# vasil-pashov/sparse_matrix_math

Hardware: AMD Instinct MI355X
Metric: CSR SpMV GB/s (% HBM peak) + BiCGStab iters/sec, 10M rows, 1/2/4/8 GPU (higher is better)
Workload: dtype f32

## Files before the change

### include/smm_hip.h

```cpp
#ifndef SMM_HIP_H
#define SMM_HIP_H

#include <stddef.h>

#ifdef __cplusplus
extern "C" {
#endif

#define SMM_HIP_VERSION_MAJOR 0
#define SMM_HIP_VERSION_MINOR 1

#define SMM_HIP_OK 0
#define SMM_HIP_ERR_INVALID (-1)
#define SMM_HIP_ERR_HIP (-2)
#define SMM_HIP_ERR_NO_DEVICE (-3)
#define SMM_HIP_ERR_PRECOND (-4)
#define SMM_HIP_ERR_NOMEM (-5)
#define SMM_HIP_ERR_COMM (-6)

#define SMM_SOLVER_SUCCESS 0
#define SMM_SOLVER_DIVERGED 1
#define SMM_SOLVER_MAX_ITERATIONS_REACHED 2

#define SMM_OP_ASSIGN 0
// ... 3 lines not shown
#define SMM_PRECOND_NONE 0
#define SMM_PRECOND_JACOBI 1
#define SMM_PRECOND_ILU0 2
#define SMM_PRECOND_SGS 3
#define SMM_PRECOND_IC0 4
#define SMM_PRECOND_BLOCK_ILU0 5
#define SMM_PRECOND_BLOCK_SGS 6

#define SMM_DTYPE_F32 0
#define SMM_DTYPE_F64 1
#define SMM_DTYPE_I64 2

#define SMM_SPMV_AUTO 0
#define SMM_SPMV_VECTOR 1
#define SMM_SPMV_STREAM 2
#define SMM_SPMV_PATTERN 3
#define SMM_PATTERN_NONE 0
#define SMM_PATTERN_MASKS 1
#define SMM_PATTERN_CODES 2
#define SMM_PATTERN_CONST 3

typedef struct smm_hip_csr smm_hip_csr;
typedef struct smm_hip_precond smm_hip_precond;
typedef void* smm_hip_stream;

int smm_hip_init(int device);
int smm_hip_shutdown(void);
const char* smm_hip_last_error(void);
int smm_hip_uses_std_fma(void);
int smm_hip_device_info(char* name, size_t name_cap, int* cus, size_t* hbm_bytes);
int smm_hip_stream_synchronize(smm_hip_stream stream);

int smm_hip_debug_fail_next_alloc(size_t min_bytes);
int smm_hip_profile_enable(int on);
int smm_hip_profile_read(double* spmv_ms, long long* spmv_launches, int reset);
int smm_hip_profile_read_waits(double* exposed_ms, long long* pairs, int reset);

int smm_hip_csr_create_f32(int rows, int cols, const int* start, const int* positions, const float* values, smm_hip_csr** out);
int smm_hip_csr_create_f64(int rows, int cols, const int* start, const int* positions, const double* values, smm_hip_csr** out);
int smm_hip_csr_create_dev_f32(int rows, int cols, const int* d_start, const int* d_positions, const float* d_values, smm_hip_csr** out);
int smm_hip_csr_create_dev_f64(int rows, int cols, const int* d_start, const int* d_positions, const double* d_values, smm_hip_csr** out);
int smm_hip_csr_destroy(smm_hip_csr* m);
int smm_hip_csr_info(const smm_hip_csr* m, int* rows, int* cols, int* nnz, int* dtype, int* first_active_start);
int smm_hip_csr_set_kernel(smm_hip_csr* m, int family, int lanes_per_row);
int smm_hip_csr_get_kernel(const smm_hip_csr* m, int* family, int* lanes_per_row);
int smm_hip_csr_tile_info(const smm_hip_csr* m, int* tiles, int* tile_nnz_cap, int* tile_max_rows, int* tile_kernel);
int smm_hip_csr_pattern_info(const smm_hip_csr* m, int* encoding, int* offsets);
int smm_hip_csr_kernel_desc(const smm_hip_csr* m, char* name, int name_cap, long long* bytes_per_launch);
int smm_hip_set_march_min_rows(long long const_diagonals_rows, long long values_read_rows);
int smm_hip_set_cg_lazy_x_min_bytes(long long bytes);
int smm_hip_set_cg_fuse_p(int on);
int smm_hip_csr_pattern_allow_const(smm_hip_csr* m, int allow);
int smm_hip_csr_pattern_slots(smm_hip_csr* m, int mode);
int smm_hip_csr_autotune(smm_hip_csr* m);

#define SMM_UPDATE_SET 0
#define SMM_UPDATE_ADD 1
int smm_hip_csr_scale_f32(smm_hip_csr* m, float alpha, smm_hip_stream stream);
int smm_hip_csr_scale_f64(smm_hip_csr* m, double alpha, smm_hip_stream stream);
int smm_hip_csr_axpy_f32(smm_hip_csr* m, float alpha, const smm_hip_csr* other, smm_hip_stream stream);
int smm_hip_csr_axpy_f64(smm_hip_csr* m, double alpha, const smm_hip_csr* other, smm_hip_stream stream);
int smm_hip_csr_zero_f32(smm_hip_csr* m, smm_hip_stream stream);
int smm_hip_csr_zero_f64(smm_hip_csr* m, smm_hip_stream stream);
int smm_hip_csr_update_entries_f32(smm_hip_csr* m, int n, const int* rows, const int* cols, const float* values, int mode, unsigned char* found);
int smm_hip_csr_update_entries_f64(smm_hip_csr* m, int n, const int* rows, const int* cols, const double* values, int mode, unsigned char* found);
int smm_hip_csr_update_entries_dev_f32(smm_hip_csr* m, int n, const int* d_rows, const int* d_cols, const float* d_values, int mode, unsigned char* d_found,
                                       smm_hip_stream stream);
int smm_hip_csr_update_entries_dev_f64(smm_hip_csr* m, int n, const int* d_rows, const int* d_cols, const double* d_values, int mode, unsigned char* d_found,
                                       smm_hip_stream stream);
int smm_hip_csr_set_values_f32(smm_hip_csr* m, const float* values);
int smm_hip_csr_set_values_f64(smm_hip_csr* m, const double* values);
int smm_hip_csr_set_values_dev_f32(smm_hip_csr* m, const float* d_values, smm_hip_stream stream);
int smm_hip_csr_set_values_dev_f64(smm_hip_csr* m, const double* d_values, smm_hip_stream stream);
int smm_hip_csr_get_values_f32(const smm_hip_csr* m, float* values);
int smm_hip_csr_get_values_f64(const smm_hip_csr* m, double* values);
int smm_hip_csr_values_changed_f32(smm_hip_csr* m, smm_hip_stream stream);
int smm_hip_csr_values_changed_f64(smm_hip_csr* m, smm_hip_stream stream);
int smm_hip_csr_same_pattern(const smm_hip_csr* a, const smm_hip_csr* b, int* same);

int smm_hip_spmv_f32(const smm_hip_csr* m, int op, const float* lhs, const float* x, float* out);
int smm_hip_spmv_f64(const smm_hip_csr* m, int op, const double* lhs, const double* x, double* out);
int smm_hip_spmv_dev_f32(const smm_hip_csr* m, int op, const float* d_lhs, const float* d_x, float* d_out, smm_hip_stream stream);
int smm_hip_spmv_dev_f64(const smm_hip_csr* m, int op, const double* d_lhs, const double* d_x, double* d_out, smm_hip_stream stream);

int smm_hip_dot_f32(int n, const float* a, const float* b, float* result);
int smm_hip_dot_f64(int n, const double* a, const double* b, double* result);
int smm_hip_dot_dev_f32(int n, const float* d_a, const float* d_b, float* d_result, smm_hip_stream stream);
int smm_hip_dot_dev_f64(int n, const double* d_a, const double* d_b, double* d_result, smm_hip_stream stream);

int smm_hip_axpy_dev_f32(int n, float a, const float* d_x, const float* d_y, float* d_out, smm_hip_stream stream);
int smm_hip_axpy_dev_f64(int n, double a, const double* d_x, const double* d_y, double* d_out, smm_hip_stream stream);

int smm_hip_cg_f32(const smm_hip_csr* a, const float* b, const float* x0, float* x, int maxIterations, float eps,
                   const smm_hip_precond* M, int* solver_status, int* iterations, float* resnorm2);
int smm_hip_cg_f64(const smm_hip_csr* a, const double* b, const double* x0, double* x, int maxIterations, double eps,
                   const smm_hip_precond* M, int* solver_status, int* iterations, double* resnorm2);
int smm_hip_cg_dev_f32(const smm_hip_csr* a, const float* d_b, const float* d_x0, float* d_x, int maxIterations, float eps,
                       const smm_hip_precond* M, smm_hip_stream stream, int* solver_status, int* iterations, float* resnorm2);
int smm_hip_cg_dev_f64(const smm_hip_csr* a, const double* d_b, const double* d_x0, double* d_x, int maxIterations, double eps,
                       const smm_hip_precond* M, smm_hip_stream stream, int* solver_status, int* iterations, double* resnorm2);

#define SMM_CG_RESIDENT_OFF 0
#define SMM_CG_RESIDENT_AUTO 1
#define SMM_CG_RESIDENT_REQUIRE 2
int smm_hip_cg_resident(int mode);

// ... 157 lines not shown
```

### sparse_matrix_math_amd/_lib.py

```python
import ctypes
import os
from ctypes import POINTER, c_char_p, c_double, c_float, c_int, c_longlong, c_size_t, c_ulonglong, c_void_p

_HERE = os.path.dirname(os.path.abspath(__file__))

SMM_HIP_OK = 0
SMM_HIP_ERR_INVALID = -1
SMM_HIP_ERR_HIP = -2
SMM_HIP_ERR_NO_DEVICE = -3
SMM_HIP_ERR_PRECOND = -4
SMM_HIP_ERR_NOMEM = -5
SMM_HIP_ERR_COMM = -6


class SmmHipError(RuntimeError):
    def __init__(self, code, message):
        super().__init__(f"libsmm_hip error {code}: {message}")
        self.code = code


def library_path(fma=False):
    if os.environ.get("SMM_HIP_LIBRARY"):
        return os.environ["SMM_HIP_LIBRARY"]
    name = "libsmm_hip_fma.so" if fma else "libsmm_hip.so"
# ... 26 lines not shown
    "smm_hip_precond_apply_spmv_dev": (c_int, [_P, _P, _P, _P]),
    "smm_hip_precond_values": (c_int, [_P, _P, c_size_t]),
    "smm_hip_gen_poisson2d_dev": (c_int, [c_int, c_int, _P, _P, _P, _P]),
    "smm_hip_gen_stencil3d_dev": (c_int, [c_int, c_int, c_int, "T", "T", "T", _P, _P, _P, _P]),
    "smm_hip_gen_banded_dev": (c_int, [c_int, c_int, c_ulonglong, c_int, "T", _P, _P, _P, _P]),
    "smm_hip_gen_banded_rows_dev": (c_int, [c_int, c_int, c_ulonglong, c_int, "T", c_int, c_int, _P, _P, _P, _P]),
    "smm_hip_spmv_fused_dev": (c_int, [_P, c_int, _P, _P, _P, c_int, _P, _P, _P]),
    "smm_hip_spmv_fused_finish_dev": (c_int, [_P, c_int, _P, _P, _P, c_int, _P, _P, _P]),
    "smm_hip_bicgstab_ws_create": (c_int, [c_int, POINTER(_P)]),
    "smm_hip_bicgstab_ws_stage": (c_int, [_P, c_int, _P, "T", _P]),
    "smm_hip_cg_ws_stage": (c_int, [_P, c_int, _P, _P, "T", _P]),
    "smm_hip_bicgstab_ws_result": (c_int, [_P, _P, POINTER(c_int), POINTER(c_int), "PT"]),
    "smm_hip_dist_csr_create_dev": (c_int, [_P, c_int, POINTER(c_int), _P, _P, _P, POINTER(_P)]),
    "smm_hip_dist_spmv_dev": (c_int, [_P, c_int, _P, _P, _P, _P]),
    "smm_hip_dist_bicgstab_dev": (c_int, [_P, _P, _P, c_int, "T", _P, _P, POINTER(c_int), POINTER(c_int), "PT"]),
    "smm_hip_dist_cg_dev": (c_int, [_P, _P, _P, _P, c_int, "T", _P, POINTER(c_int), POINTER(c_int), "PT"]),
    "smm_hip_csr_scale": (c_int, [_P, "T", _P]),
    "smm_hip_csr_axpy": (c_int, [_P, "T", _P, _P]),
    "smm_hip_csr_zero": (c_int, [_P, _P]),
    "smm_hip_csr_update_entries": (c_int, [_P, c_int, _P, _P, _P, c_int, _P]),
    "smm_hip_csr_update_entries_dev": (c_int, [_P, c_int, _P, _P, _P, c_int, _P, _P]),
    "smm_hip_csr_set_values": (c_int, [_P, _P]),
    "smm_hip_csr_set_values_dev": (c_int, [_P, _P, _P]),
    "smm_hip_csr_get_values": (c_int, [_P, _P]),
    "smm_hip_csr_values_changed": (c_int, [_P, _P]),
}



_PLAIN = {
    "smm_hip_init": (c_int, [c_int]),
    "smm_hip_shutdown": (c_int, []),
    "smm_hip_last_error": (c_char_p, []),
    "smm_hip_uses_std_fma": (c_int, []),
    "smm_hip_device_info": (c_int, [c_char_p, c_size_t, POINTER(c_int), POINTER(c_size_t)]),
    "smm_hip_stream_synchronize": (c_int, [_P]),
    "smm_hip_debug_fail_next_alloc": (c_int, [c_size_t]),
    "smm_hip_profile_enable": (c_int, [c_int]),
    "smm_hip_profile_read": (c_int, [POINTER(c_double), POINTER(c_longlong), c_int]),
    "smm_hip_profile_read_waits": (c_int, [POINTER(c_double), POINTER(c_longlong), c_int]),
    "smm_hip_csr_destroy": (c_int, [_P]),
    "smm_hip_csr_info": (c_int, [_P, POINTER(c_int), POINTER(c_int), POINTER(c_int), POINTER(c_int), POINTER(c_int)]),
    "smm_hip_csr_set_kernel": (c_int, [_P, c_int, c_int]),
    "smm_hip_csr_get_kernel": (c_int, [_P, POINTER(c_int), POINTER(c_int)]),
    "smm_hip_csr_autotune": (c_int, [_P]),
    "smm_hip_csr_tile_info": (c_int, [_P, POINTER(c_int), POINTER(c_int), POINTER(c_int), POINTER(c_int)]),
    "smm_hip_csr_pattern_info": (c_int, [_P, POINTER(c_int), POINTER(c_int)]),
    "smm_hip_csr_kernel_desc": (c_int, [_P, c_char_p, c_int, POINTER(c_longlong)]),
    "smm_hip_set_march_min_rows": (c_int, [c_longlong, c_longlong]),
    "smm_hip_set_cg_lazy_x_min_bytes": (c_int, [c_longlong]),
    "smm_hip_set_cg_fuse_p": (c_int, [c_int]),
    "smm_hip_csr_pattern_allow_const": (c_int, [_P, c_int]),
    "smm_hip_csr_pattern_slots": (c_int, [_P, c_int]),
    "smm_hip_csr_same_pattern": (c_int, [_P, _P, POINTER(c_int)]),
    "smm_hip_precond_create": (c_int, [_P, c_int, POINTER(_P)]),
    "smm_hip_precond_create_block": (c_int, [_P, c_int, c_int, POINTER(_P)]),
    "smm_hip_precond_create_block_capped": (c_int, [_P, c_int, c_int, c_int, POINTER(_P)]),
    "smm_hip_precond_block_level_cap": (c_int, [_P, POINTER(c_int)]),
    "smm_hip_precond_create_block_ex": (c_int, [_P, c_int, c_int, c_int, c_int, POINTER(_P)]),
    "smm_hip_precond_block_rows": (c_int, [_P, _P, c_size_t, _P]),
    "smm_hip_precond_block_record_bytes": (c_int, [_P, POINTER(c_int), POINTER(c_int), POINTER(c_int)]),
    "smm_hip_precond_block_count": (c_int, [_P, POINTER(c_int)]),
    "smm_hip_precond_block_bounds": (c_int, [_P, _P, c_size_t]),
    "smm_hip_precond_destroy": (c_int, [_P]),
    "smm_hip_precond_set_sweep": (c_int, [_P, c_int]),
    "smm_hip_precond_take_error": (c_int, [_P, _P]),
    "smm_hip_precond_info": (c_int, [_P, POINTER(c_int), POINTER(c_int), POINTER(c_int)]),
    "smm_hip_gen_poisson2d_nnz": (c_longlong, [c_int, c_int]),
    "smm_hip_gen_stencil3d_nnz": (c_longlong, [c_int, c_int, c_int]),
    "smm_hip_gen_banded_nnz": (c_longlong, [c_int, c_int, c_ulonglong, c_int]),
    "smm_hip_gen_banded_row_start": (c_longlong, [c_int, c_int, c_ulonglong, c_int, c_int]),
    "smm_hip_partials_count": (c_int, []),
    "smm_hip_finish_len": (c_int, []),
    "smm_hip_finish_totals_offset": (c_int, []),
    "smm_hip_cg_resident": (c_int, [c_int]),
    "smm_hip_bicgstab_resident": (c_int, [c_int]),
    "smm_hip_bicgstab_ws_destroy": (c_int, [_P]),
    "smm_hip_cg_ws_status": (c_int, [_P, _P, POINTER(c_int)]),
    "smm_hip_bicgstab_ws_bind": (c_int, [_P, _P, _P, _P]),
    "smm_hip_bicgstab_ws_pointers": (c_int, [_P, POINTER(_P), POINTER(_P), POINTER(_P), POINTER(_P), POINTER(_P), POINTER(_P)]),
    "smm_hip_comm_unique_id": (c_int, [_P]),
    "smm_hip_comm_create_rccl": (c_int, [c_int, c_int, _P, POINTER(_P)]),
    "smm_hip_comm_create_host": (c_int, [c_int, c_int, HOST_ALLREDUCE_FN, HOST_SENDRECV_FN, _P, POINTER(_P)]),
    "smm_hip_comm_create_self": (c_int, [POINTER(_P)]),
    "smm_hip_comm_destroy": (c_int, [_P]),
    "smm_hip_comm_info": (c_int, [_P, POINTER(c_int), POINTER(c_int), POINTER(c_int)]),
    "smm_hip_comm_selftest": (c_int, [_P]),
    "smm_hip_comm_rccl_ranks": (c_int, [_P, POINTER(c_int)]),
    "smm_hip_partition_rows_by_nnz": (c_int, [_P, c_int, c_int, _P]),
    "smm_hip_dist_csr_destroy": (c_int, [_P]),
    "smm_hip_dist_csr_info": (c_int, [_P, POINTER(c_int), POINTER(c_int), POINTER(c_int), POINTER(c_int), POINTER(c_longlong), POINTER(c_longlong)]),
    "smm_hip_dist_csr_local_block": (c_int, [_P, POINTER(_P), POINTER(_P)]),
    "smm_hip_dist_csr_halo_chunks": (c_int, [_P, POINTER(c_int)]),
    "smm_hip_dist_csr_options": (c_int, [_P, POINTER(c_int), POINTER(c_int), POINTER(c_int), POINTER(ctypes.c_double)]),
    "smm_hip_dist_csr_matvec_forms": (c_int, [_P, POINTER(ctypes.c_longlong), POINTER(ctypes.c_longlong)]),
    "smm_hip_dist_csr_thin_remote": (c_int, [_P, POINTER(c_int), POINTER(ctypes.c_longlong)]),
    "smm_hip_dist_csr_cg_fused": (c_int, [_P, POINTER(ctypes.c_longlong)]),
    "smm_hip_dist_csr_split_wait": (c_int, [_P, POINTER(ctypes.c_double), c_int]),
    "smm_hip_dist_p2p_plan": (c_int, [c_int, c_int, POINTER(c_longlong), POINTER(c_int), c_int, c_double, POINTER(c_longlong), c_int, POINTER(c_int)]),
}


def exported_symbols():
    names = list(_PLAIN)
    for base in _TYPED:
        names += [f"{base}_f32", f"{base}_f64"]
# ... 66 lines not shown
```

### sparse_matrix_math_amd/csrc/smm_internal.h

```cpp
#pragma once
#include <hip/hip_runtime.h>

#include <cstddef>
#include <cstdint>
#include <cstdio>
#include <atomic>
#include <chrono>
#include <cstdlib>
#include <cstring>
#include <mutex>
#include <string>
#include <type_traits>
#include <vector>

#include "../../include/smm_hip.h"

namespace smm {

void setError(const char* fmt, ...);
int hipFail(hipError_t e, const char* what, const char* file, int line);

#define SMM_HIP_TRY(expr)                                             \
	do {                                                              \
		hipError_t _e = (expr);                                       \
// ... 73 lines not shown
		n = 0;
	}
	T* detach() {
		T* q = p;
		p = nullptr;
		n = 0;
		return q;
	}
	operator T*() const { return p; }
};

template <typename T>
constexpr int dtypeOf() { return std::is_same<T, float>::value ? SMM_DTYPE_F32 : SMM_DTYPE_F64; }

}

struct smm_hip_csr {
	int rows = 0, cols = 0, nnz = 0, dtype = 0;
	int firstActiveStart = 0;
	bool ready = false;
	bool kernelForced = false;
	std::mutex readyMutex;
	int* d_start = nullptr;
	int* d_positions = nullptr;
	void* d_values = nullptr;
	bool owns = false;
	std::atomic<int> kernelWord{SMM_SPMV_VECTOR | (4 << 8)};
	int family() const { return kernelWord.load(std::memory_order_acquire) & 0xFF; }
	int lanes() const { return kernelWord.load(std::memory_order_acquire) >> 8; }
	void setKernel(int family, int lanes) { kernelWord.store((family & 0xFF) | (lanes << 8), std::memory_order_release); }
	std::mutex adoptMutex;
	int* d_rowblocks = nullptr;
	int n_rowblocks = 0;
	int stream_nnz_cap = 0;
	int stream_max_rows = 0;
	int stream_chunk_tiles = 0;
	int stream_mid_len = 0;
	int max_row_len = -1;
	std::mutex tileMutex;
	std::atomic<int> pat_state{0};
	int pat_encoding = 0;
	unsigned short* d_pat_codes = nullptr;
	bool pat_const = false;
	unsigned long long* d_pat_cval = nullptr;
	std::vector<unsigned long long> pat_cval_host;
	void* d_res_ell = nullptr;
	bool pat_const_off = false;
	void* d_pat_slots = nullptr;
	long long* d_pat_slot_base = nullptr;
	int pat_slots_state = 0;
	int pat_slots_mode = -1;
	long long pat_slots_elems = 0;
	int pat_slots_waves = 0, pat_slots_uniform = 0;
	int pat_max_off = 0;
	bool march_ok = false;
	int march_P = 0, march_H = 0, march_lo = 0, march_hi = 0;
	bool march_clusters = false;
	unsigned* d_pat_masks32 = nullptr;
	unsigned char* d_pat_masks8 = nullptr;
	std::vector<int> pat_offs_host;
	int pat_k = 0;
	int* d_pat_off = nullptr;
	unsigned long long* d_pat_masks = nullptr;
	int* d_pat_rowblocks = nullptr;
	int pat_n_rowblocks = 0;
	int pat_nnz_cap = 0;
	int pat_max_rows = 0;
	int pat_chunk_tiles = 0;
	int split_tile_max[3] = {-1, -1, -1};
	bool split_uneven = false;
	std::atomic<unsigned long long> uid{0};
	std::mutex editMutex;
	std::vector<std::pair<unsigned long long, bool>> patternSeen;
};

struct smm_hip_precond {
	int kind = SMM_PRECOND_NONE;
	int dtype = 0;
	const smm_hip_csr* a = nullptr;
	void* d_values = nullptr;
	size_t n_values = 0;
	int* d_order_lo = nullptr;
	int* d_order_up = nullptr;
	std::vector<int> lvl_ptr_lo, lvl_ptr_up;
	struct smm_precond_plan* plan = nullptr;
	struct smm_precond_block* blk = nullptr;
};

namespace smm {

constexpr int NPART = 2048;

template <typename T>
int launchSpmv(const smm_hip_csr* m, int op, const T* lhs, const T* x, T* out, int dotMode, const T* w1, T* partials,
               const int* doneFlag, hipStream_t s, int extraFlags = 0, const T* divisor = nullptr);

int profBegin(hipStream_t s);
void profEnd(int slot, hipStream_t s);
int profWaitAwaited(hipStream_t awaited);
void profWaitWaiting(int slot, hipStream_t waiting);

constexpr int SPMV_NT_OUT = 0x100;
constexpr int SPMV_FINISH = 0x200;
constexpr int SPMV_LEAVE_ROOM = 0x400;
constexpr int SPMV_DIV_LHS = 0x800;
constexpr int SPMV_OP_DIV = 3;
constexpr int SPMV_ADD_DIV = 0x1000;
constexpr int SPMV_OP_ADD_DIV = 4;
constexpr int SPMV_HALF_TILES = 0x2000;
constexpr int SPMV_NO_FULL_ROWS = 0x4000;
constexpr int PARTS_TOTALS = 2 * NPART;
constexpr int PARTS_TICKETS = 16;
constexpr int PARTS_LEN = 2 * NPART + 2 + 2 * (PARTS_TICKETS + 1);
template <typename T>
__host__ __device__ inline unsigned* partsTicket(T* partials) { return reinterpret_cast<unsigned*>(partials + PARTS_TOTALS + 2); }
inline int spmvOutFlags(const smm_hip_csr* m, size_t elemBytes) {
	static const int forced = [] {
		const char* env = getenv("SMM_HIP_NT_OUT");
		return env ? atoi(env) : -1;
	}();
	if (forced >= 0) return forced ? SPMV_NT_OUT : 0;
	return static_cast<double>(m->rows) * static_cast<double>(elemBytes) >= 64.0 * 1024 * 1024 ? SPMV_NT_OUT : 0;
}

int buildRowBlocks(smm_hip_csr* m, int capNnz, int maxRows, hipStream_t s);
int buildTileTable(const smm_hip_csr* m, int capNnz, int maxRows, hipStream_t s, int** blocks, int* nBlocks, int* chunkTiles);
int cutRows(const int* d_start, int rows, long long nnz, int capNnz, int maxRows, hipStream_t s, int2** tiles, int* nTiles, int tilesPerChunk = 0);
int ensureCsrReady(const smm_hip_csr* m, hipStream_t s, bool streamKnown);
int ensurePattern(smm_hip_csr* m, hipStream_t s = nullptr, bool streamKnown = false, bool quiet = false, bool masksOnly = false);
int adoptPatternForSolver(const smm_hip_csr* m, int plannedIterations, hipStream_t s);
void adoptPatternQuietly(const smm_hip_csr* m, hipStream_t s);
int patternLanesFor(const smm_hip_csr* m);
const char* patternKernelDesc(const smm_hip_csr* m, int lanes, long long* bytes);
void planMarch(smm_hip_csr* m);
int refreshResEll(smm_hip_csr* a, hipStream_t s);
bool ensurePatternSlots(smm_hip_csr* m, int lanes, hipStream_t s);
bool patternSlotsChosen(const smm_hip_csr* m, int lanes);
long long patternSlotsBytes(const smm_hip_csr* m);
int refreshPatternSlots(smm_hip_csr* m, hipStream_t s);
int marchBuildMasks32(smm_hip_csr* m, hipStream_t s);
template <typename K>
inline int occupancyCached(std::atomic<long long>& slot, K kernel, int tpb, size_t lds, int fallback) {
	const long long seen = slot.load(std::memory_order_acquire);
	if (seen != 0 && static_cast<size_t>(seen >> 8) == lds) return static_cast<int>(seen & 0xFF);
	int n = 0;
	if (hipOccupancyMaxActiveBlocksPerMultiprocessor(&n, kernel, tpb, lds) != hipSuccess || n < 1) {
		(void)hipGetLastError();
		n = fallback;
	}
	n = n > 255 ? 255 : n;
	slot.store((static_cast<long long>(lds) << 8) | n, std::memory_order_release);
	return n;
}
template <typename K>
inline bool ensureDynamicLds(std::atomic<int>& granted, K kernel, size_t lds) {
	if (lds <= 64 * 1024) return true;
	int have = granted.load(std::memory_order_acquire);
	while (static_cast<size_t>(have) < lds) {
		if (hipFuncSetAttribute(reinterpret_cast<const void*>(kernel), hipFuncAttributeMaxDynamicSharedMemorySize, static_cast<int>(lds)) != hipSuccess) {
			(void)hipGetLastError();
			return false;
		}
		if (granted.compare_exchange_weak(have, static_cast<int>(lds), std::memory_order_acq_rel)) break;
	}
	return true;
}
inline int forcedWgsPerCU() {
	static const int forced = [] {
		const char* env = getenv("SMM_HIP_STREAM_WGS_PER_CU");
		return env ? (atoi(env) > 1 ? atoi(env) : 1) : 0;
	}();
	return forced;
}

bool cgHalfTiles(const smm_hip_csr* m, size_t elemBytes);
long long cgLazyMinBytes();
bool updateNT(long long n, size_t elemBytes, int vectors);
bool masksMarchApplies(const smm_hip_csr* m);
bool constMarchApplies(const smm_hip_csr* m);
template <typename T>
bool launchPatMasksMarch(const smm_hip_csr* m, int op, const T* lhs, const T* divisor, const T* x, T* out, int dotMode, const T* w1, T* partials,
                         const int* doneFlag, hipStream_t s);
template <typename T>
bool launchPatConstMarch(const smm_hip_csr* m, int op, const T* lhs, const T* divisor, const T* x, T* out, int dotMode, const T* w1, T* partials,
                         const int* doneFlag, hipStream_t s);
template <typename T>
void launchPatSlots(const smm_hip_csr* m, int lanes, int op, const T* lhs, const T* divisor, const T* x, T* out, int dotMode, const T* w1, T* partials,
                    const int* doneFlag, hipStream_t s);
template <typename T>
int launchSpmvPattern(const smm_hip_csr* m, int lanes, int op, const T* lhs, const T* divisor, const T* x, T* out, int dotMode, const T* w1, T* partials,
                      const int* doneFlag, hipStream_t s);
// ... 130 lines not shown
```

### sparse_matrix_math_amd/csrc/smm_spmv_slots.hip

```cpp
#include <algorithm>

#include <rocprim/device/device_scan.hpp>

#include "smm_pattern_dev.h"

namespace smm {

constexpr int SLOT_WAVES = TPB / WAVE;

__global__ __launch_bounds__(TPB) void slotsCountKernel(int rows, int nWaves, const unsigned long long* __restrict__ masks, long long* __restrict__ counts,
                                                        int* __restrict__ uniformWaves) {
	const int lane = threadIdx.x & (WAVE - 1);
	int mine = 0;
	for (int w = (blockIdx.x * TPB + threadIdx.x) / WAVE; w < nWaves; w += gridDim.x * SLOT_WAVES) {
		const int row = w * WAVE + lane;
		const unsigned long long mm = row < rows ? masks[row] : ~0ULL;
		const unsigned long long lead = patUniform64(mm);
		const bool uniform = lead != 0ULL && __builtin_amdgcn_ballot_w64(!(row < rows && mm == lead)) == 0ULL;
		if (lane == 0) {
			counts[w] = uniform ? static_cast<long long>(__builtin_popcountll(lead)) * WAVE : 0;
			mine += uniform;
		}
	}
	if (lane == 0 && mine) atomicAdd(uniformWaves, mine);
}

__global__ __launch_bounds__(TPB) void slotsMarkKernel(int nWaves, const long long* __restrict__ counts, long long* __restrict__ base) {
	for (int w = blockIdx.x * TPB + threadIdx.x; w < nWaves; w += gridDim.x * TPB) {
		if (counts[w] == 0) base[w] = -1;
	}
}

template <typename T>
__global__ __launch_bounds__(TPB) void slotsFillKernel(int nWaves, const long long* __restrict__ base, const unsigned long long* __restrict__ masks,
                                                       const int* __restrict__ start, const T* __restrict__ values, T* __restrict__ slots) {
	const int lane = threadIdx.x & (WAVE - 1);
	for (int w = (blockIdx.x * TPB + threadIdx.x) / WAVE; w < nWaves; w += gridDim.x * SLOT_WAVES) {
		const long long b = base[w];
		if (b < 0) continue;
		const int row = w * WAVE + lane;
		const int len = __builtin_popcountll(masks[w * WAVE]);
		const T* src = values + start[row];
		T* dst = slots + b + lane;
		for (int e = 0; e < len; ++e) dst[static_cast<long long>(e) * WAVE] = src[e];
	}
}

template <typename T, int L, int G>
__global__ __launch_bounds__(TPB) void spmvPatternSlotsKernel(int rows, int nWaves, int chunkWaves, const int* __restrict__ offs,
                                                              const long long* __restrict__ base, const unsigned long long* __restrict__ masks,
                                                              const T* __restrict__ slots, const int* __restrict__ start, const int* __restrict__ positions,
                                                              const T* __restrict__ values, int opFlags, const T* lhs, const T* __restrict__ divisor,
                                                              const T* __restrict__ x, T* out, int dotMode, const T* __restrict__ w1,
// ... 6 lines not shown
	const int t = threadIdx.x;
	const int lane = t & (WAVE - 1);
	const int wave = __builtin_amdgcn_readfirstlane(t >> 6);
	const int nGroups = min(8, static_cast<int>(gridDim.x));
	const int xcdGroup = blockIdx.x % nGroups;
	const int groupSlots = (static_cast<int>(gridDim.x) - xcdGroup + nGroups - 1) / nGroups;
	const int wEnd = min(nWaves, (xcdGroup + 1) * chunkWaves);
	T acc0 = T(0), acc1 = T(0);
	for (int w = xcdGroup * chunkWaves + static_cast<int>(blockIdx.x / nGroups) * SLOT_WAVES + wave; w < wEnd; w += groupSlots * SLOT_WAVES) {
		const int row = w * WAVE + lane;
		const long long b = base[w];
		T dot = T(0);
		if (b >= 0) {
			const unsigned long long lead = masks[w * WAVE];
			const int len = __builtin_popcountll(lead);
			const int pl = (len + L - 1) / L;
			const int offLane = offs[lane < len ? selectBit(lead, lane) : 0];
			const T* const xr = x + row;
			const T* const sv = slots + b + lane;
			T part[L];
#pragma unroll
			for (int q = 0; q < L; ++q) part[q] = T(0);
			for (int i = 0; i < pl; i += G) {
				T vv[L][G], xv[L][G];
#pragma unroll
				for (int q = 0; q < L; ++q) {
#pragma unroll
					for (int u = 0; u < G; ++u) {
						const int e = min(q * pl + i + u, len - 1);
						vv[q][u] = __builtin_nontemporal_load(sv + static_cast<long long>(e) * WAVE);
						xv[q][u] = xr[__builtin_amdgcn_readlane(offLane, e)];
					}
				}
#pragma unroll
				for (int q = 0; q < L; ++q) {
#pragma unroll
					for (int u = 0; u < G; ++u) {
						if (i + u < pl && q * pl + i + u < len) part[q] = smmFma(vv[q][u], xv[q][u], part[q]);
					}
				}
			}
			dot = part[0];
#pragma unroll
			for (int q = 1; q < L; ++q) dot += part[q];
		} else if (row < rows) {
			dot = patRowDirect<T, L>(start[row], start[row + 1], values, positions, x);
		}
		if (row < rows) {
			const T o = patApplyOp(op, lhs, divisor, row, dot);
			storeOut(out + row, o, ntOut);
			if (dotMode == 2) acc0 += o * o;
			if (dotMode) acc1 += o * w1[row];
		}
	}
	if (dotMode) {
		if (dotMode == 2) {
			const T s0 = blockSum256(acc0, red);
			if (t == 0) partials[blockIdx.x] = s0;
		}
		const T s1 = blockSum256(acc1, red);
		if (t == 0) partials[(dotMode == 2 ? NPART : 0) + blockIdx.x] = s1;
		for (int i = gridDim.x + blockIdx.x * TPB + t; i < NPART; i += gridDim.x * TPB) {
			partials[i] = T(0);
			if (dotMode == 2) partials[NPART + i] = T(0);
		}
		if (opFlags & SPMV_FINISH) lastBlockSums<T>(partials, NPART, dotMode == 2 ? 2 : 1, partials + PARTS_TOTALS, partsTicket(partials));
	}
}

static int slotsEnvMode() {
	static const int mode = [] {
		const char* env = getenv("SMM_HIP_PATTERN_SLOTS");
		return env ? (atoi(env) != 0 ? 1 : 0) : -1;
	}();
	return mode;
}

static int slotsMode(const smm_hip_csr* m) { return m->pat_slots_mode >= 0 ? m->pat_slots_mode : slotsEnvMode(); }

static bool slotsApplies(const smm_hip_csr* m, int lanes) {
	if (lanes != 2 && lanes != 4) return false;
	if (m->pat_encoding != 0 || (m->pat_const && !m->pat_const_off)) return false;
	static const bool fullRows = [] {
		const char* env = getenv("SMM_HIP_FULL_ROWS");
		const char* variant = getenv("SMM_HIP_PATTERN_VARIANT");
		return !(env && atoi(env) == 0) && !(variant && atoi(variant) == 0);
	}();
	return fullRows;
}

static bool slotsWanted(const smm_hip_csr* m, int lanes, bool* forced) {
	const int mode = slotsMode(m);
	*forced = mode == 1;
	if (mode == 0 || !slotsApplies(m, lanes)) return false;
	return mode == 1 || mode == 2 || !m->kernelForced;
}

static bool slotsUniformEnough(const smm_hip_csr* m) {
	return static_cast<long long>(m->pat_slots_uniform) * 100 >= static_cast<long long>(m->pat_slots_waves) * 99;
}

bool patternSlotsChosen(const smm_hip_csr* m, int lanes) {
	bool forced = false;
	if (!slotsWanted(m, lanes, &forced) || m->pat_slots_state != 1 || !m->d_pat_slots) return false;
	return forced || slotsUniformEnough(m);
}
// ... 34 lines not shown
	SMM_HIP_TRY(hipMemcpyAsync(&total, base.p + nWaves, sizeof(total), hipMemcpyDeviceToHost, s));
	SMM_HIP_TRY(hipMemcpyAsync(&nUniform, uniform.p, sizeof(nUniform), hipMemcpyDeviceToHost, s));
	SMM_HIP_TRY(hipStreamSynchronize(s));
	m->pat_slots_waves = nWaves;
	m->pat_slots_uniform = nUniform;
	m->pat_slots_elems = total;
	if (!forced && !slotsUniformEnough(m)) return SMM_HIP_ERR_INVALID;
	const size_t bytes = static_cast<size_t>(std::max(1LL, total)) * sizeof(T);
	size_t freeB = 0, totalB = 0;
	SMM_HIP_TRY(hipMemGetInfo(&freeB, &totalB));
	if (freeB < bytes + std::max<size_t>(size_t(1) << 30, totalB / 16)) return SMM_HIP_ERR_INVALID;
	void* p = nullptr;
	SMM_TRY(devAlloc(&p, bytes));
	m->d_pat_slots = p;
	m->d_pat_slot_base = base.detach();
	int st = slotsFill<T>(m, s);
	hipError_t e = st == SMM_HIP_OK ? hipStreamSynchronize(s) : hipSuccess;
	if (st != SMM_HIP_OK || e != hipSuccess) {
		devFree(m->d_pat_slots);
		devFree(m->d_pat_slot_base);
		m->d_pat_slots = nullptr;
		m->d_pat_slot_base = nullptr;
		return st != SMM_HIP_OK ? st : hipFail(e, "slotsFillKernel", __FILE__, __LINE__);
	}
	return SMM_HIP_OK;
}

bool ensurePatternSlots(smm_hip_csr* m, int lanes, hipStream_t s) {
	bool forced = false;
	if (!slotsWanted(m, lanes, &forced)) return false;
	if (m->pat_slots_state == 1 && m->d_pat_slots) return forced || slotsUniformEnough(m);
	if (m->pat_slots_state < 0 && !forced) return false;
	const int st = m->dtype == SMM_DTYPE_F32 ? slotsBuild<float>(m, forced, s) : slotsBuild<double>(m, forced, s);
	if (st != SMM_HIP_OK) {
		m->pat_slots_state = -1;
		(void)hipGetLastError();
		setError("");
		return false;
	}
	m->pat_slots_state = 1;
	return true;
}

int refreshPatternSlots(smm_hip_csr* m, hipStream_t s) {
	if (!m->d_pat_slots || !m->d_pat_slot_base || m->rows <= 0) return SMM_HIP_OK;
	return m->dtype == SMM_DTYPE_F32 ? slotsFill<float>(m, s) : slotsFill<double>(m, s);
}

long long patternSlotsBytes(const smm_hip_csr* m) {
	const long long s = m->dtype == SMM_DTYPE_F32 ? 4 : 8;
	const long long rows = m->rows, nnz = m->nnz;
	const long long otherRows = std::max(0LL, rows - 64LL * m->pat_slots_uniform);
	const long long otherNnz = std::max(0LL, nnz - m->pat_slots_elems);
	return m->pat_slots_elems * s + static_cast<long long>(m->pat_slots_waves) * 16 + otherNnz * (s + 4) + (otherRows + m->pat_slots_waves) * 4 +
	       static_cast<long long>(m->cols) * s + rows * s;
}

static int slotsBatch(const smm_hip_csr* m, int lanes) {
	const long long len = m->pat_slots_uniform > 0 ? (m->pat_slots_elems + 32LL * m->pat_slots_uniform) / (64LL * m->pat_slots_uniform) : 1;
	const int p = static_cast<int>(std::max(1LL, (len + lanes - 1) / lanes));
	const int nb = (p + 15) / 16;
	const int g = (p + nb - 1) / nb;
	return g <= 8 ? 8 : g <= 13 ? 13 : 16;
}

template <typename T, int L, int G>
static void launchSlotsG(const smm_hip_csr* m, int op, const T* lhs, const T* divisor, const T* x, T* out, int dotMode, const T* w1, T* partials,
                         const int* doneFlag, hipStream_t s) {
	static std::atomic<long long> occ{0};
	const int perCU = occupancyCached(occ, spmvPatternSlotsKernel<T, L, G>, TPB, 0, 4);
	const int cus = (op & SPMV_LEAVE_ROOM) ? std::max(8, numCUs() - 8) : numCUs();
	const int nWaves = m->pat_slots_waves;
	const int grid = std::max(1, std::min(std::min((nWaves + SLOT_WAVES - 1) / SLOT_WAVES, cus * perCU), NPART));
	const int nGroups = std::min(8, grid);
	const int chunkWaves = (nWaves + nGroups - 1) / nGroups;
	spmvPatternSlotsKernel<T, L, G><<<grid, TPB, 0, s>>>(m->rows, nWaves, chunkWaves, m->d_pat_off, m->d_pat_slot_base, m->d_pat_masks,
	                                                    static_cast<const T*>(m->d_pat_slots), m->d_start, m->d_positions, static_cast<const T*>(m->d_values),
	                                                    (op & ~SPMV_LEAVE_ROOM) | spmvOutFlags(m, sizeof(T)), lhs, divisor, x, out, dotMode, w1, partials,
	                                                    doneFlag);
}

template <typename T, int L>
static void launchSlotsL(const smm_hip_csr* m, int op, const T* lhs, const T* divisor, const T* x, T* out, int dotMode, const T* w1, T* partials,
                         const int* doneFlag, hipStream_t s) {
	switch (slotsBatch(m, L)) {
	case 8: launchSlotsG<T, L, 8>(m, op, lhs, divisor, x, out, dotMode, w1, partials, doneFlag, s); break;
	case 13: launchSlotsG<T, L, 13>(m, op, lhs, divisor, x, out, dotMode, w1, partials, doneFlag, s); break;
	default: launchSlotsG<T, L, 16>(m, op, lhs, divisor, x, out, dotMode, w1, partials, doneFlag, s); break;
	}
}

template <typename T>
void launchPatSlots(const smm_hip_csr* m, int lanes, int op, const T* lhs, const T* divisor, const T* x, T* out, int dotMode, const T* w1, T* partials,
                    const int* doneFlag, hipStream_t s) {
	if (lanes == 2) {
		launchSlotsL<T, 2>(m, op, lhs, divisor, x, out, dotMode, w1, partials, doneFlag, s);
	} else {
		launchSlotsL<T, 4>(m, op, lhs, divisor, x, out, dotMode, w1, partials, doneFlag, s);
	}
}

template void launchPatSlots<float>(const smm_hip_csr*, int, int, const float*, const float*, const float*, float*, int, const float*, float*, const int*,
                                    hipStream_t);
template void launchPatSlots<double>(const smm_hip_csr*, int, int, const double*, const double*, const double*, double*, int, const double*, double*,
                                     const int*, hipStream_t);

}

extern "C" int smm_hip_csr_pattern_slots(smm_hip_csr* m, int mode) {
	if (!m || mode < -1 || mode > 2) {
		smm::setError("csr_pattern_slots: null matrix or a mode other than -1, 0, 1, 2");
		return SMM_HIP_ERR_INVALID;
	}
	std::lock_guard<std::mutex> lock(m->tileMutex);
	m->pat_slots_mode = mode;
	if (mode == 1 && m->pat_slots_state < 0) m->pat_slots_state = 0;
	return SMM_HIP_OK;
}
```

### sparse_matrix_math_amd/host.py

```python
import ctypes
import enum

import numpy as np

from . import _lib
from ._lib import check


class SolverStatus(enum.IntEnum):
    SUCCESS = 0
    DIVERGED = 1
    MAX_ITERATIONS_REACHED = 2


class SolverPreconditioner(enum.IntEnum):
    NONE = 0
    JACOBI = 1
    ILU0 = 2
    SYMMETRIC_GAUS_SEIDEL = 3
    IC0 = 4
    BLOCK_ILU0 = 5
    BLOCK_SGS = 6


# ... 215 lines not shown
        return self.nnz

    def set_kernel(self, family=SPMV_AUTO, lanes_per_row=0):
        check(_lib.load().smm_hip_csr_set_kernel(self._h, int(family), int(lanes_per_row)))

    def get_kernel(self):
        fam, lanes = ctypes.c_int(), ctypes.c_int()
        check(_lib.load().smm_hip_csr_get_kernel(self._h, ctypes.byref(fam), ctypes.byref(lanes)))
        return fam.value, lanes.value

    def autotune(self):
        check(_lib.load().smm_hip_csr_autotune(self._h))
        return self.get_kernel()

    def _spmv(self, op, lhs, mult, out):
        fn = _fn("smm_hip_spmv", self._suf)
        plhs = _host(lhs, self.dtype, "lhs", self.rows) if op != OP_ASSIGN else ctypes.c_void_p(0)
        check(fn(self._h, op, plhs, _host(mult, self.dtype, "mult", self.cols), _host(out, self.dtype, "out", self.rows, True)))

    def rMult(self, mult, res):
        self._spmv(OP_ASSIGN, None, mult, res)

    def rMultAdd(self, lhs, mult, out):
        self._spmv(OP_ADD, lhs, mult, out)

    def rMultSub(self, lhs, mult, out):
        self._spmv(OP_SUB, lhs, mult, out)

    def spmv_dev(self, op, d_lhs, d_x, d_out, stream=None):
        check(_fn("smm_hip_spmv_dev", self._suf)(self._h, int(op), _dptr(d_lhs), _dptr(d_x), _dptr(d_out), _dptr(stream)))

    def tile_info(self):
        v = [ctypes.c_int() for _ in range(4)]
        check(_lib.load().smm_hip_csr_tile_info(self._h, *[ctypes.byref(c) for c in v]))
        return tuple(c.value for c in v)

    def pattern_info(self):
        enc, k = ctypes.c_int(), ctypes.c_int()
        check(_lib.load().smm_hip_csr_pattern_info(self._h, ctypes.byref(enc), ctypes.byref(k)))
        return enc.value, k.value

    def kernel_desc(self):
        buf = ctypes.create_string_buffer(64)
        nbytes = ctypes.c_longlong()
        check(_lib.load().smm_hip_csr_kernel_desc(self._h, buf, 64, ctypes.byref(nbytes)))
        return buf.value.decode(), nbytes.value

    def pattern_allow_const(self, allow):
        check(_lib.load().smm_hip_csr_pattern_allow_const(self._h, 1 if allow else 0))

    def pattern_slots(self, mode):
        check(_lib.load().smm_hip_csr_pattern_slots(self._h, int(mode)))

    def _edited(self, stream):
        if stream is None:
            synchronize(None)

    def scale(self, alpha, stream=None):
        check(_fn("smm_hip_csr_scale", self._suf)(self._h, float(alpha), _dptr(stream)))
        self._edited(stream)

    def axpy(self, alpha, other, stream=None):
        check(_fn("smm_hip_csr_axpy", self._suf)(self._h, float(alpha), other._h, _dptr(stream)))
        self._edited(stream)

    def zero(self, stream=None):
        check(_fn("smm_hip_csr_zero", self._suf)(self._h, _dptr(stream)))
        self._edited(stream)

    def __imul__(self, alpha):
        self.scale(alpha)
        return self

    def inplaceAdd(self, other):
        self.axpy(1.0, other)

    def inplaceSubtract(self, other):
        self.axpy(-1.0, other)

    def zeroValues(self):
        self.zero()

    def hasSameNonZeroPattern(self, other):
        same = ctypes.c_int()
        check(_lib.load().smm_hip_csr_same_pattern(self._h, other._h, ctypes.byref(same)))
        return bool(same.value)

    def update_entries(self, rows, cols, vals, add=False):
        rows = np.ascontiguousarray(rows, dtype=np.int32)
        cols = np.ascontiguousarray(cols, dtype=np.int32)
        vals = np.ascontiguousarray(vals, dtype=self.dtype)
        n = rows.size
        if cols.size != n or vals.size != n:
            raise ValueError("rows, cols and vals must have the same length")
        found = np.zeros(n, dtype=np.uint8)
        check(_fn("smm_hip_csr_update_entries", self._suf)(self._h, n, _host(rows, np.int32, "rows"), _host(cols, np.int32, "cols"), _host(vals, self.dtype, "vals"),
                                                          1 if add else 0, _host(found, np.uint8, "found")))
        return found.astype(bool)

    def update_entries_dev(self, n, d_rows, d_cols, d_vals, add=False, d_found=None, stream=None):
        check(_fn("smm_hip_csr_update_entries_dev", self._suf)(self._h, int(n), _dptr(d_rows), _dptr(d_cols), _dptr(d_vals), 1 if add else 0, _dptr(d_found),
                                                              _dptr(stream)))
        self._edited(stream)

    def updateEntry(self, row, col, value):
        return bool(self.update_entries([row], [col], [value])[0])
# ... 156 lines not shown
```

Measured before the change: 908.3.

## Add multi-pass pattern-slots SpMV kernel splitting diagonals into L2-friendly passes

```diff
diff --git a/include/smm_hip.h b/include/smm_hip.h
--- a/include/smm_hip.h
+++ b/include/smm_hip.h
@@ -79,6 +79,7 @@
 int smm_hip_set_cg_fuse_p(int on);
 int smm_hip_csr_pattern_allow_const(smm_hip_csr* m, int allow);
 int smm_hip_csr_pattern_slots(smm_hip_csr* m, int mode);
+int smm_hip_csr_pattern_passes(smm_hip_csr* m, int passes);
 int smm_hip_csr_autotune(smm_hip_csr* m);
 
 #define SMM_UPDATE_SET 0
diff --git a/sparse_matrix_math_amd/_lib.py b/sparse_matrix_math_amd/_lib.py
--- a/sparse_matrix_math_amd/_lib.py
+++ b/sparse_matrix_math_amd/_lib.py
@@ -102,6 +102,7 @@
     "smm_hip_set_cg_fuse_p": (c_int, [c_int]),
     "smm_hip_csr_pattern_allow_const": (c_int, [_P, c_int]),
     "smm_hip_csr_pattern_slots": (c_int, [_P, c_int]),
+    "smm_hip_csr_pattern_passes": (c_int, [_P, c_int]),
     "smm_hip_csr_same_pattern": (c_int, [_P, _P, POINTER(c_int)]),
     "smm_hip_precond_create": (c_int, [_P, c_int, POINTER(_P)]),
     "smm_hip_precond_create_block": (c_int, [_P, c_int, c_int, POINTER(_P)]),
diff --git a/sparse_matrix_math_amd/csrc/smm_internal.h b/sparse_matrix_math_amd/csrc/smm_internal.h
--- a/sparse_matrix_math_amd/csrc/smm_internal.h
+++ b/sparse_matrix_math_amd/csrc/smm_internal.h
@@ -149,6 +149,7 @@
 	int pat_slots_mode = -1;
 	long long pat_slots_elems = 0;
 	int pat_slots_waves = 0, pat_slots_uniform = 0;
+	int pat_passes_mode = -1;
 	int pat_max_off = 0;
 	bool march_ok = false;
 	int march_P = 0, march_H = 0, march_lo = 0, march_hi = 0;
@@ -234,6 +235,8 @@
 bool ensurePatternSlots(smm_hip_csr* m, int lanes, hipStream_t s);
 bool patternSlotsChosen(const smm_hip_csr* m, int lanes);
 long long patternSlotsBytes(const smm_hip_csr* m);
+int patternSlotsPasses(const smm_hip_csr* m, int lanes);
+int slotsPassesModel(const std::vector<int>& offs, int lanes, int elemBytes);
 int refreshPatternSlots(smm_hip_csr* m, hipStream_t s);
 int marchBuildMasks32(smm_hip_csr* m, hipStream_t s);
 template <typename K>
diff --git a/sparse_matrix_math_amd/csrc/smm_spmv_slots.hip b/sparse_matrix_math_amd/csrc/smm_spmv_slots.hip
--- a/sparse_matrix_math_amd/csrc/smm_spmv_slots.hip
+++ b/sparse_matrix_math_amd/csrc/smm_spmv_slots.hip
@@ -1,4 +1,5 @@
 #include <algorithm>
+#include <utility>
 
 #include <rocprim/device/device_scan.hpp>
 
@@ -111,6 +112,103 @@
 			if (dotMode == 2) acc0 += o * o;
 			if (dotMode) acc1 += o * w1[row];
 		}
+	}
+	if (dotMode) {
+		if (dotMode == 2) {
+			const T s0 = blockSum256(acc0, red);
+			if (t == 0) partials[blockIdx.x] = s0;
+		}
+		const T s1 = blockSum256(acc1, red);
+		if (t == 0) partials[(dotMode == 2 ? NPART : 0) + blockIdx.x] = s1;
+		for (int i = gridDim.x + blockIdx.x * TPB + t; i < NPART; i += gridDim.x * TPB) {
+			partials[i] = T(0);
+			if (dotMode == 2) partials[NPART + i] = T(0);
+		}
+		if (opFlags & SPMV_FINISH) lastBlockSums<T>(partials, NPART, dotMode == 2 ? 2 : 1, partials + PARTS_TOTALS, partsTicket(partials));
+	}
+}
+
+template <int... Rs, typename F>
+__device__ __forceinline__ void slotsForEachRow(std::integer_sequence<int, Rs...>, F&& f) {
+	(f(std::integral_constant<int, Rs>{}), ...);
+}
+
+template <typename T, int L, int G, int R>
+__global__ __launch_bounds__(TPB) void spmvPatternSlotsPassKernel(int rows, int nWaves, int chunkWaves, int passes, const int* __restrict__ offs,
+                                                                  const long long* __restrict__ base, const unsigned long long* __restrict__ masks,
+                                                                  const T* __restrict__ slots, const int* __restrict__ start, const int* __restrict__ positions,
+                                                                  const T* __restrict__ values, int opFlags, const T* lhs, const T* __restrict__ divisor,
+                                                                  const T* __restrict__ x, T* out, int dotMode, const T* __restrict__ w1,
+                                                                  T* __restrict__ partials, const int* __restrict__ doneFlag) {
+	static_assert(L == 2 || L == 4, "pieces per row");
+	__shared__ T red[4];
+	if (doneFlag && *doneFlag) return;
+	const int op = opFlags & 0xFF;
+	const bool ntOut = (opFlags & SPMV_NT_OUT) != 0;
+	const int t = threadIdx.x;
+	const int lane = t & (WAVE - 1);
+	const int wave = __builtin_amdgcn_readfirstlane(t >> 6);
+	const int nGroups = min(8, static_cast<int>(gridDim.x));
+	const int xcdGroup = blockIdx.x % nGroups;
+	const int groupSlots = (static_cast<int>(gridDim.x) - xcdGroup + nGroups - 1) / nGroups;
+	const int wEnd = min(nWaves, (xcdGroup + 1) * chunkWaves);
+	const int w0 = xcdGroup * chunkWaves + static_cast<int>(blockIdx.x / nGroups) * SLOT_WAVES + wave;
+	const int stride = groupSlots * SLOT_WAVES;
+	T acc0 = T(0), acc1 = T(0);
+	T carry[R][L];
+#pragma unroll
+	for (int r = 0; r < R; ++r) {
+#pragma unroll
+		for (int q = 0; q < L; ++q) carry[r][q] = T(0);
+	}
+	for (int p = 0; p < passes; ++p) {
+		const bool last = p == passes - 1;
+		slotsForEachRow(std::make_integer_sequence<int, R>{}, [&](auto rc) {
+			constexpr int r = decltype(rc)::value;
+			int w = w0 + r * stride;
+			asm volatile("" : "+s"(w));
+			const bool mine = w < wEnd;
+			const int row = w * WAVE + lane;
+			const long long b = mine ? base[w] : -1;
+			if (b >= 0) {
+				const unsigned long long lead = masks[w * WAVE];
+				const int len = __builtin_popcountll(lead);
+				const int pl = (len + L - 1) / L;
+				const int lo = pl * p / passes, hi = pl * (p + 1) / passes;
+				const int offLane = offs[lane < len ? selectBit(lead, lane) : 0];
+				const T* const xr = x + row;
+				const T* const sv = slots + b + lane;
+				for (int i = lo; i < hi; i += G) {
+					T vv[L][G], xv[L][G];
+#pragma unroll
+					for (int q = 0; q < L; ++q) {
+#pragma unroll
+						for (int u = 0; u < G; ++u) {
+							const int e = min(q * pl + min(i + u, hi - 1), len - 1);
+							vv[q][u] = __builtin_nontemporal_load(sv + static_cast<long long>(e) * WAVE);
+							xv[q][u] = xr[__builtin_amdgcn_readlane(offLane, e)];
+						}
+					}
+#pragma unroll
+					for (int q = 0; q < L; ++q) {
+#pragma unroll
+						for (int u = 0; u < G; ++u) {
+							if (i + u < hi && q * pl + i + u < len) carry[r][q] = smmFma(vv[q][u], xv[q][u], carry[r][q]);
+						}
+					}
+				}
+			}
+			if (last && mine && row < rows) {
+				T dot = carry[r][0];
+#pragma unroll
+				for (int q = 1; q < L; ++q) dot += carry[r][q];
+				if (b < 0) dot = patRowDirect<T, L>(start[row], start[row + 1], values, positions, x);
+				const T o = patApplyOp(op, lhs, divisor, row, dot);
+				storeOut(out + row, o, ntOut);
+				if (dotMode == 2) acc0 += o * o;
+				if (dotMode) acc1 += o * w1[row];
+			}
+		});
 	}
 	if (dotMode) {
 		if (dotMode == 2) {
@@ -251,7 +349,8 @@
 	const long long rows = m->rows, nnz = m->nnz;
 	const long long otherRows = std::max(0LL, rows - 64LL * m->pat_slots_uniform);
 	const long long otherNnz = std::max(0LL, nnz - m->pat_slots_elems);
-	return m->pat_slots_elems * s + static_cast<long long>(m->pat_slots_waves) * 16 + otherNnz * (s + 4) + (otherRows + m->pat_slots_waves) * 4 +
+	const long long headers = std::max(1, patternSlotsPasses(m, std::min(m->kernelWord.load(std::memory_order_acquire) >> 8, WAVE)));
+	return m->pat_slots_elems * s + static_cast<long long>(m->pat_slots_waves) * 16 * headers + otherNnz * (s + 4) + (otherRows + m->pat_slots_waves) * 4 +
 	       static_cast<long long>(m->cols) * s + rows * s;
 }
 
@@ -279,9 +378,113 @@
 	                                                    doneFlag);
 }
 
+constexpr int PASS_CARRY_REGS = 104;
+constexpr int PASS_BATCH_REGS = 14;
+constexpr int PASS_MAX = 8;
+
+template <typename T, int L>
+constexpr int passRows() {
+	return PASS_CARRY_REGS * 4 / (L * static_cast<int>(sizeof(T)));
+}
+
+template <typename T, int L>
+constexpr int passBatch() {
+	return std::max(1, PASS_BATCH_REGS * 4 / (L * static_cast<int>(sizeof(T))));
+}
+
+constexpr double PASS_L2_BYTES = 4.0 * 1024 * 1024;
+constexpr double PASS_COST_BYTES = 4.0;
+
+int slotsPassesModel(const std::vector<int>& offs, int lanes, int elemBytes) {
+	const int len = static_cast<int>(offs.size());
+	const int pl = (len + lanes - 1) / lanes;
+	if (pl < 2) return 0;
+	double best = 0.0;
+	int bestP = 1;
+	for (int P = 1; P <= std::min(PASS_MAX, pl); ++P) {
+		double misses = 0.0;
+		for (int p = 0; p < P; ++p) {
+			const int lo = pl * p / P, hi = pl * (p + 1) / P;
+			std::vector<int> g;
+			for (int q = 0; q < lanes; ++q) {
+				for (int i = lo; i < hi && q * pl + i < len; ++i) g.push_back(offs[q * pl + i]);
+			}
+			if (g.empty()) continue;
+			const double inflow = static_cast<double>(g.size() + lanes) * elemBytes;
+			misses += 1.0;
+			for (size_t j = 1; j < g.size(); ++j) {
+				if (static_cast<double>(g[j] - g[j - 1]) * inflow > PASS_L2_BYTES) misses += 1.0;
+			}
+		}
+		const double bytes = misses * elemBytes + (P - 1) * PASS_COST_BYTES;
+		if (P == 1 || bytes < best) {
+			best = bytes;
+			bestP = P;
+		}
+	}
+	return bestP > 1 ? bestP : 0;
+}
+
+static int passesEnvMode() {
+	static const int mode = [] {
+		const char* env = getenv("SMM_HIP_PATTERN_PASSES");
+		return env ? std::max(0, std::min(PASS_MAX, atoi(env))) : -1;
+	}();
+	return mode;
+}
+
+static int slotsGrid(const smm_hip_csr* m, int op, int perCU) {
+	const int cus = (op & SPMV_LEAVE_ROOM) ? std::max(8, numCUs() - 8) : numCUs();
+	return std::max(1, std::min(std::min((m->pat_slots_waves + SLOT_WAVES - 1) / SLOT_WAVES, cus * perCU), NPART));
+}
+
+static int slotsRowsPerWave(int nWaves, int grid) {
+	const int nGroups = std::min(8, grid);
+	const int chunkWaves = (nWaves + nGroups - 1) / nGroups;
+	const int waves = grid / nGroups * SLOT_WAVES;
+	return (chunkWaves + waves - 1) / waves;
+}
+
+template <typename T, int L>
+static int slotsPassPlan(const smm_hip_csr* m, int op, int* grid) {
+	const int mode = m->pat_passes_mode >= 0 ? m->pat_passes_mode : passesEnvMode();
+	const int passes = mode >= 0 ? mode : slotsPassesModel(m->pat_offs_host, L, static_cast<int>(sizeof(T)));
+	if (passes <= 0) return 0;
+	static std::atomic<long long> occ{0};
+	const int perCU = occupancyCached(occ, spmvPatternSlotsPassKernel<T, L, passBatch<T, L>(), passRows<T, L>()>, TPB, 0, 3);
+	*grid = slotsGrid(m, op, perCU);
+	return slotsRowsPerWave(m->pat_slots_waves, *grid) <= passRows<T, L>() ? passes : 0;
+}
+
+int patternSlotsPasses(const smm_hip_csr* m, int lanes) {
+	int grid = 0;
+	const bool f32 = m->dtype == SMM_DTYPE_F32;
+	if (lanes == 2) return f32 ? slotsPassPlan<float, 2>(m, 0, &grid) : slotsPassPlan<double, 2>(m, 0, &grid);
+	if (lanes == 4) return f32 ? slotsPassPlan<float, 4>(m, 0, &grid) : slotsPassPlan<double, 4>(m, 0, &grid);
+	return 0;
+}
+
+template <typename T, int L>
+static void launchSlotsPass(const smm_hip_csr* m, int passes, int grid, int op, const T* lhs, const T* divisor, const T* x, T* out, int dotMode,
+                            const T* w1, T* partials, const int* doneFlag, hipStream_t s) {
+	const int nWaves = m->pat_slots_waves;
+	const int nGroups = std::min(8, grid);
+	const int chunkWaves = (nWaves + nGroups - 1) / nGroups;
+	spmvPatternSlotsPassKernel<T, L, passBatch<T, L>(), passRows<T, L>()><<<grid, TPB, 0, s>>>(
+	    m->rows, nWaves, chunkWaves, passes, m->d_pat_off, m->d_pat_slot_base, m->d_pat_masks, static_cast<const T*>(m->d_pat_slots), m->d_start,
+	    m->d_positions, static_cast<const T*>(m->d_values), (op & ~SPMV_LEAVE_ROOM) | spmvOutFlags(m, sizeof(T)), lhs, divisor, x, out, dotMode, w1,
+	    partials, doneFlag);
+}
+
 template <typename T, int L>
 static void launchSlotsL(const smm_hip_csr* m, int op, const T* lhs, const T* divisor, const T* x, T* out, int dotMode, const T* w1, T* partials,
                          const int* doneFlag, hipStream_t s) {
+	int grid = 0;
+	const int passes = slotsPassPlan<T, L>(m, op, &grid);
+	if (passes > 0) {
+		launchSlotsPass<T, L>(m, passes, grid, op, lhs, divisor, x, out, dotMode, w1, partials, doneFlag, s);
+		return;
+	}
 	switch (slotsBatch(m, L)) {
 	case 8: launchSlotsG<T, L, 8>(m, op, lhs, divisor, x, out, dotMode, w1, partials, doneFlag, s); break;
 	case 13: launchSlotsG<T, L, 13>(m, op, lhs, divisor, x, out, dotMode, w1, partials, doneFlag, s); break;
@@ -316,3 +519,13 @@
 	if (mode == 1 && m->pat_slots_state < 0) m->pat_slots_state = 0;
 	return SMM_HIP_OK;
 }
+
+extern "C" int smm_hip_csr_pattern_passes(smm_hip_csr* m, int passes) {
+	if (!m || passes < -1 || passes > smm::PASS_MAX) {
+		smm::setError("csr_pattern_passes: null matrix or a pass count other than -1 .. 8");
+		return SMM_HIP_ERR_INVALID;
+	}
+	std::lock_guard<std::mutex> lock(m->tileMutex);
+	m->pat_passes_mode = passes;
+	return SMM_HIP_OK;
+}
diff --git a/sparse_matrix_math_amd/host.py b/sparse_matrix_math_amd/host.py
--- a/sparse_matrix_math_amd/host.py
+++ b/sparse_matrix_math_amd/host.py
@@ -291,6 +291,9 @@
     def pattern_slots(self, mode):
         check(_lib.load().smm_hip_csr_pattern_slots(self._h, int(mode)))
 
+    def pattern_passes(self, passes):
+        check(_lib.load().smm_hip_csr_pattern_passes(self._h, int(passes)))
+
     def _edited(self, stream):
         if stream is None:
             synchronize(None)
```

New measurement: 586.0 (median of 2 runs). 0.645x the previous value.
